# Project-MONAI/GenerativeModels

Hardware: NVIDIA H100
Metric: ddim50_voxels_per_s (higher is better)
Workload: dtype fp16

## Files before the change

generativemodels_b200/csrc/flash_attn.cu:

```cuda
#include "common.cuh"
#include "wgmma.cuh"
#include <cuda.h>
#include <cudaTypedefs.h>
#include <mutex>
#include <string.h>

namespace b200 {

struct FlashDev {
  alignas(64) CUtensorMap tmQ;
  alignas(64) CUtensorMap tmK;
  alignas(64) CUtensorMap tmVt;
  int B, T, S, heads, dh, d_chunks;
  int q_tiles, q_tiles_grid, n_items, n_kv;
  float scale_log2;
  h16* out;
  long long out_bstride, out_pitch;
  const h16* res;
  long long res_bstride, res_pitch;
};

namespace fa {

static constexpr int kThreads = 128;
static constexpr int kBM = 64, kBKV = 64;
static constexpr int kChunkBytes = 64 * 64 * 2;

__device__ __forceinline__ float ex2_approx(float x) {
  float y;
  asm("ex2.approx.ftz.f32 %0, %1;" : "=f"(y) : "f"(x));
  return y;
}
__device__ __forceinline__ uint32_t pack_h2(float lo, float hi) {
  h162 v = f2h2(lo, hi);
  return *reinterpret_cast<uint32_t*>(&v);
}

template <int DCH>
__global__ void __launch_bounds__(kThreads, 1) flash_attn_kernel(const __grid_constant__ FlashDev p) {
  constexpr int DV = 64 * DCH;
  extern __shared__ uint8_t smem_raw[];
  const uint32_t q_base = (smem_u32(smem_raw) + 1023u) & ~1023u;
  const uint32_t k_base = q_base + DCH * kChunkBytes;
  const uint32_t v_base = k_base + DCH * kChunkBytes;
  const uint32_t bar = v_base + DV * kBKV * 2;
  const uint32_t q_bar = bar, k_bar = bar + 8, v_bar = bar + 16;

  const int tid = threadIdx.x;
  const int warp = tid >> 5, lane = tid & 31;
  int x = blockIdx.x;
  const int qt = x % p.q_tiles; x /= p.q_tiles;
  const int h = x % p.heads;
  const int b = x / p.heads;
  const int q0 = qt * kBM;
  const int qc = h * p.dh;
  const int vc = qc;

  if (tid == 0) {
    mbar_init(q_bar, 1);
    mbar_init(k_bar, 1);
    mbar_init(v_bar, 1);
    asm volatile("fence.mbarrier_init.release.cluster;" ::: "memory");
    asm volatile("fence.proxy.async.shared::cta;" ::: "memory");
  }
  __syncthreads();
  if (tid == 0) {
    mbar_arrive_expect_tx(q_bar, DCH * kChunkBytes);
    for (int c = 0; c < DCH; ++c) tma_load_3d(&p.tmQ, q_bar, q_base + c * kChunkBytes, qc + 64 * c, q0, b);
    mbar_arrive_expect_tx(k_bar, DCH * kChunkBytes);
    for (int c = 0; c < DCH; ++c) tma_load_3d(&p.tmK, k_bar, k_base + c * kChunkBytes, qc + 64 * c, 0, b);
    mbar_arrive_expect_tx(v_bar, DV * kBKV * 2);
    tma_load_3d(&p.tmVt, v_bar, v_base, 0, vc, b);
  }

  float o[DV / 2];
#pragma unroll
  for (int i = 0; i < DV / 2; ++i) o[i] = 0.f;
  float m0 = -INFINITY, m1 = -INFINITY, l0 = 0.f, l1 = 0.f;
  const float sc = p.scale_log2;
  mbar_wait(q_bar, 0);

  for (int j = 0; j < p.n_kv; ++j) {
    const uint32_t ph = j & 1;
    float s[32];
    mbar_wait(k_bar, ph);
    wgmma_fence();
#pragma unroll
    for (int c = 0; c < DCH; ++c) {
      const uint64_t qd = wgmma_desc(q_base + c * kChunkBytes), kd = wgmma_desc(k_base + c * kChunkBytes);
#pragma unroll
      for (int kk = 0; kk < 4; ++kk) wgmma_ss<64>(s, qd + 2u * kk, kd + 2u * kk, (c | kk) != 0 ? 1u : 0u);
    }
    wgmma_commit();
    wgmma_wait<0>();
    wgmma_touch<32>(s);
    __syncthreads();
    if (tid == 0 && j + 1 < p.n_kv) {
      mbar_arrive_expect_tx(k_bar, DCH * kChunkBytes);
      for (int c = 0; c < DCH; ++c) tma_load_3d(&p.tmK, k_bar, k_base + c * kChunkBytes, qc + 64 * c, (j + 1) * kBKV, b);
    }

    const int key0 = j * kBKV + 2 * (lane & 3);
    float mx0 = -INFINITY, mx1 = -INFINITY;
#pragma unroll
    for (int n = 0; n < 8; ++n) {
#pragma unroll
      for (int e = 0; e < 2; ++e) {
        const bool ok = key0 + 8 * n + e < p.S;
        s[4 * n + e] = ok ? s[4 * n + e] * sc : -INFINITY;
        s[4 * n + 2 + e] = ok ? s[4 * n + 2 + e] * sc : -INFINITY;
        mx0 = fmaxf(mx0, s[4 * n + e]);
        mx1 = fmaxf(mx1, s[4 * n + 2 + e]);
      }
    }
    mx0 = fmaxf(mx0, __shfl_xor_sync(0xffffffffu, mx0, 1));
    mx0 = fmaxf(mx0, __shfl_xor_sync(0xffffffffu, mx0, 2));
    mx1 = fmaxf(mx1, __shfl_xor_sync(0xffffffffu, mx1, 1));
    mx1 = fmaxf(mx1, __shfl_xor_sync(0xffffffffu, mx1, 2));
    const float nm0 = fmaxf(m0, mx0), nm1 = fmaxf(m1, mx1);
    const float u0 = nm0 == -INFINITY ? 0.f : nm0, u1 = nm1 == -INFINITY ? 0.f : nm1;
    const float a0 = ex2_approx(m0 - u0), a1 = ex2_approx(m1 - u1);
    m0 = nm0;
    m1 = nm1;
    uint32_t pa[16];
    float ps0 = 0.f, ps1 = 0.f;
#pragma unroll
    for (int n = 0; n < 8; ++n) {
      const float p00 = ex2_approx(s[4 * n] - u0), p01 = ex2_approx(s[4 * n + 1] - u0);
      const float p10 = ex2_approx(s[4 * n + 2] - u1), p11 = ex2_approx(s[4 * n + 3] - u1);
      ps0 += p00 + p01;
      ps1 += p10 + p11;
      pa[4 * (n >> 1) + 2 * (n & 1)] = pack_h2(p00, p01);
      pa[4 * (n >> 1) + 2 * (n & 1) + 1] = pack_h2(p10, p11);
    }
    l0 = l0 * a0 + ps0;
    l1 = l1 * a1 + ps1;
#pragma unroll
    for (int n = 0; n < DV / 8; ++n) {
      o[4 * n] *= a0; o[4 * n + 1] *= a0;
      o[4 * n + 2] *= a1; o[4 * n + 3] *= a1;
    }

    mbar_wait(v_bar, ph);
    wgmma_fence();
    const uint64_t vd = wgmma_desc(v_base);
#pragma unroll
    for (int kk = 0; kk < 4; ++kk) wgmma_rs<DV>(o, pa + 4 * kk, vd + 2u * kk, 1u);
    wgmma_commit();
    wgmma_wait<0>();
    wgmma_touch<DV / 2>(o);
    __syncthreads();
    if (tid == 0 && j + 1 < p.n_kv) {
      mbar_arrive_expect_tx(v_bar, DV * kBKV * 2);
      tma_load_3d(&p.tmVt, v_bar, v_base, (j + 1) * kBKV, vc, b);
    }
  }

  l0 += __shfl_xor_sync(0xffffffffu, l0, 1);
  l0 += __shfl_xor_sync(0xffffffffu, l0, 2);
  l1 += __shfl_xor_sync(0xffffffffu, l1, 1);
  l1 += __shfl_xor_sync(0xffffffffu, l1, 2);
  const float inv0 = 1.f / l0, inv1 = 1.f / l1;
  const int r0 = 16 * warp + (lane >> 2);
#pragma unroll
  for (int half = 0; half < 2; ++half) {
    const int t = q0 + r0 + 8 * half;
    if (t >= p.T) continue;
    const float inv = half ? inv1 : inv0;
    h16* orow = p.out + (long long)b * p.out_bstride + (long long)t * p.out_pitch + vc;
    const h16* rrow = p.res ? p.res + (long long)b * p.res_bstride + (long long)t * p.res_pitch + vc : nullptr;
#pragma unroll
    for (int n = 0; n < DV / 8; ++n) {
      const int col = 8 * n + 2 * (lane & 3);
      float v0 = o[4 * n + 2 * half] * inv, v1 = o[4 * n + 2 * half + 1] * inv;
      if (rrow) {
        const float2 r = h22f2(*reinterpret_cast<const h162*>(rrow + col));
        v0 += r.x;
        v1 += r.y;
      }
      *reinterpret_cast<h162*>(orow + col) = f2h2(v0, v1);
    }
  }
}

template <int DCH>
constexpr int smem_bytes() { return 1024 + 2 * DCH * kChunkBytes + DCH * 64 * kBKV * 2 + 64; }

namespace d512 {
static constexpr int kThreads = 384;
static constexpr int kCluster = 2;
static constexpr int kBlockKeys = 128;
static constexpr int kRing = 16;
static constexpr int kChunksPerBlock = 32;
static constexpr int kOffRing = 8 * kChunkBytes;
static constexpr int kOffP = kOffRing + kRing * kChunkBytes;
static constexpr int kOffX = kOffP + 2 * kChunkBytes;
static constexpr int kOffBar = kOffX + 4 * 64 * 4;
static constexpr int kSmem = 1024 + kOffBar + (1 + 2 * kRing) * 8;
static constexpr int kProducerRegs = 40, kConsumerRegs = 232;
static_assert(kProducerRegs * 128 + kConsumerRegs * 256 <= 65536, "register budget of one CTA per SM");
}

__global__ void __launch_bounds__(d512::kThreads, 1) flash_attn_d512_kernel(const __grid_constant__ FlashDev p) {
  using namespace d512;
  extern __shared__ uint8_t smem_raw[];
  uint8_t* sm = smem_raw + ((1024u - (smem_u32(smem_raw) & 1023u)) & 1023u);
  const uint32_t base = smem_u32(sm);
  const uint32_t q_base = base, ring = base + kOffRing, p_base = base + kOffP;
  float* xmax = reinterpret_cast<float*>(sm + kOffX);
  float* xsum = xmax + 2 * 64;
  const uint32_t q_bar = base + kOffBar;
  const uint32_t full0 = q_bar + 8, empty0 = full0 + 8 * kRing;

  const int tid = threadIdx.x;
  const int wg = __shfl_sync(0xffffffffu, tid >> 7, 0);
  const uint32_t rank = cluster_ctarank();
  int x = blockIdx.x;
  const int qt = x % p.q_tiles_grid; x /= p.q_tiles_grid;
  const int h = x % p.heads;
  const int b = x / p.heads;
  const bool rows_valid = qt < p.q_tiles;
  const int q0 = (rows_valid ? qt : p.q_tiles - 1) * kBM;
  const int qc = h * 512;

  if (tid == 0) {
    mbar_init(q_bar, 1);
    for (int s = 0; s < kRing; ++s) {
      mbar_init(full0 + 8 * s, 1);
      mbar_init(empty0 + 8 * s, 4 * kCluster);
    }
    asm volatile("fence.mbarrier_init.release.cluster;" ::: "memory");
  }
  cluster_sync();

  if (wg == 0) {
    setmaxnreg_dec<kProducerRegs>();
    if (tid == 0) {
      mbar_arrive_expect_tx(q_bar, 8 * kChunkBytes);
      for (int c = 0; c < 8; ++c) tma_load_3d(&p.tmQ, q_bar, q_base + c * kChunkBytes, qc + 64 * c, q0, b);
      for (int j = 0; j < p.n_kv; ++j) {
        for (int n = 0; n < kChunksPerBlock; ++n) {
          const int slot = n % kRing;
          mbar_wait(empty0 + 8 * slot, ((n / kRing) & 1) ^ 1);
          mbar_arrive_expect_tx(full0 + 8 * slot, kChunkBytes);
          if ((n & 1) != (int)rank) continue;
          const uint32_t dst = ring + slot * kChunkBytes, fb = full0 + 8 * slot;
          if (n < 16) {
            const int d = (n & 3) | ((n >> 3) << 2);
            tma_load_3d_multicast(&p.tmK, fb, dst, qc + 64 * d, j * kBlockKeys + 64 * ((n >> 2) & 1), b, 0x3);
          } else {
            const int g = (n - 16) >> 2;
            tma_load_3d_multicast(&p.tmVt, fb, dst, j * kBlockKeys + 64 * (g >> 1), qc + 256 * (g & 1) + 64 * (n & 3), b,
                                  0x3);
          }
        }
      }
    }
  } else {
    setmaxnreg_inc<kConsumerRegs>();
    const int c = wg - 1;
    const int t = tid & 127, warp = t >> 5, lane = tid & 31, q4 = lane & 3;
    const int r0 = 16 * warp + (lane >> 2);
    const int sw = r0 & 7;
    uint32_t* pmine = reinterpret_cast<uint32_t*>(sm + kOffP + c * kChunkBytes);
    const uint64_t pd_partner = wgmma_desc(p_base + (1 - c) * kChunkBytes);
    auto release = [&](int slot) {
      if (lane == 0) {
        mbar_arrive_cluster(empty0 + 8 * slot, 0);
        mbar_arrive_cluster(empty0 + 8 * slot, 1);
      }
    };

    float o[128];
#pragma unroll
    for (int i = 0; i < 128; ++i) o[i] = 0.f;
    float m0 = -INFINITY, m1 = -INFINITY, l0 = 0.f, l1 = 0.f;
    const float sc = p.scale_log2;
    mbar_wait(q_bar, 0);

    for (int j = 0; j < p.n_kv; ++j) {
      float s[32];
      auto k_slot = [c](int d) { return (d & 3) | (c << 2) | ((d >> 2) << 3); };
#pragma unroll
      for (int d = 0; d < 8; ++d) {
        const int slot = k_slot(d);
        mbar_wait(full0 + 8 * slot, 0);
        if (d == 0) wgmma_fence();
        const uint64_t qd = wgmma_desc(q_base + d * kChunkBytes), kd = wgmma_desc(ring + slot * kChunkBytes);
#pragma unroll
        for (int kk = 0; kk < 4; ++kk) wgmma_ss<64>(s, qd + 2u * kk, kd + 2u * kk, (d | kk) != 0 ? 1u : 0u);
        wgmma_commit();
        if (d >= 2) {
          wgmma_wait<2>();
          release(k_slot(d - 2));
        }
      }
      wgmma_wait<1>();
      release(k_slot(6));
      wgmma_wait<0>();
      release(k_slot(7));
      wgmma_touch<32>(s);

      const int key0 = j * kBlockKeys + 64 * c + 2 * q4;
      float mx0 = -INFINITY, mx1 = -INFINITY;
#pragma unroll
      for (int n = 0; n < 8; ++n) {
#pragma unroll
        for (int e = 0; e < 2; ++e) {
          const bool ok = key0 + 8 * n + e < p.S;
          s[4 * n + e] = ok ? s[4 * n + e] * sc : -INFINITY;
          s[4 * n + 2 + e] = ok ? s[4 * n + 2 + e] * sc : -INFINITY;
          mx0 = fmaxf(mx0, s[4 * n + e]);
          mx1 = fmaxf(mx1, s[4 * n + 2 + e]);
        }
      }
      mx0 = fmaxf(mx0, __shfl_xor_sync(0xffffffffu, mx0, 1));
      mx0 = fmaxf(mx0, __shfl_xor_sync(0xffffffffu, mx0, 2));
      mx1 = fmaxf(mx1, __shfl_xor_sync(0xffffffffu, mx1, 1));
      mx1 = fmaxf(mx1, __shfl_xor_sync(0xffffffffu, mx1, 2));
      if (q4 == 0) {
        xmax[64 * c + r0] = mx0;
        xmax[64 * c + r0 + 8] = mx1;
      }
      named_sync(1, 256);
      mx0 = fmaxf(mx0, xmax[64 * (1 - c) + r0]);
      mx1 = fmaxf(mx1, xmax[64 * (1 - c) + r0 + 8]);
      const float nm0 = fmaxf(m0, mx0), nm1 = fmaxf(m1, mx1);
      const float u0 = nm0 == -INFINITY ? 0.f : nm0, u1 = nm1 == -INFINITY ? 0.f : nm1;
      const float a0 = ex2_approx(m0 - u0), a1 = ex2_approx(m1 - u1);
      m0 = nm0;
      m1 = nm1;
      uint32_t pa[16];
      float ps0 = 0.f, ps1 = 0.f;
#pragma unroll
      for (int n = 0; n < 8; ++n) {
        const float p00 = ex2_approx(s[4 * n] - u0), p01 = ex2_approx(s[4 * n + 1] - u0);
        const float p10 = ex2_approx(s[4 * n + 2] - u1), p11 = ex2_approx(s[4 * n + 3] - u1);
        ps0 += p00 + p01;
        ps1 += p10 + p11;
        const uint32_t lo = pack_h2(p00, p01), hi = pack_h2(p10, p11);
        pa[4 * (n >> 1) + 2 * (n & 1)] = lo;
        pa[4 * (n >> 1) + 2 * (n & 1) + 1] = hi;
        pmine[(r0 * 128 + ((n ^ sw) << 4) + 4 * q4) >> 2] = lo;
        pmine[((r0 + 8) * 128 + ((n ^ sw) << 4) + 4 * q4) >> 2] = hi;
      }
      asm volatile("fence.proxy.async.shared::cta;" ::: "memory");
      l0 = l0 * a0 + ps0;
      l1 = l1 * a1 + ps1;
#pragma unroll
      for (int n = 0; n < 32; ++n) {
        o[4 * n] *= a0; o[4 * n + 1] *= a0;
        o[4 * n + 2] *= a1; o[4 * n + 3] *= a1;
      }
      named_sync(1, 256);

#pragma unroll
      for (int hh = 0; hh < 2; ++hh) {
        const int g = 2 * hh + c;
#pragma unroll
        for (int i = 0; i < 4; ++i) mbar_wait(full0 + 8 * (4 * g + i), 1);
        if (hh == 0) wgmma_fence();
        const uint64_t vd = wgmma_desc(ring + 4 * g * kChunkBytes);
        if (hh == c) {
#pragma unroll
          for (int kk = 0; kk < 4; ++kk) wgmma_rs<256>(o, pa + 4 * kk, vd + 2u * kk, 1u);
        } else {
#pragma unroll
          for (int kk = 0; kk < 4; ++kk) wgmma_ss<256>(o, pd_partner + 2u * kk, vd + 2u * kk, 1u);
        }
        wgmma_commit();
      }
      wgmma_wait<1>();
#pragma unroll
      for (int i = 0; i < 4; ++i) release(4 * c + i);
      wgmma_wait<0>();
      wgmma_touch<128>(o);
      wgmma_touch_u32<16>(pa);
#pragma unroll
      for (int i = 0; i < 4; ++i) release(4 * (2 + c) + i);
    }

    l0 += __shfl_xor_sync(0xffffffffu, l0, 1);
    l0 += __shfl_xor_sync(0xffffffffu, l0, 2);
    l1 += __shfl_xor_sync(0xffffffffu, l1, 1);
    l1 += __shfl_xor_sync(0xffffffffu, l1, 2);
    if (q4 == 0) {
      xsum[64 * c + r0] = l0;
      xsum[64 * c + r0 + 8] = l1;
    }
    named_sync(1, 256);
    const float inv0 = 1.f / (l0 + xsum[64 * (1 - c) + r0]), inv1 = 1.f / (l1 + xsum[64 * (1 - c) + r0 + 8]);
    const int vc = qc + 256 * c;
#pragma unroll
    for (int half = 0; half < 2; ++half) {
      const int tq = q0 + r0 + 8 * half;
      if (!rows_valid || tq >= p.T) continue;
      const float inv = half ? inv1 : inv0;
      h16* orow = p.out + (long long)b * p.out_bstride + (long long)tq * p.out_pitch + vc;
      const h16* rrow = p.res ? p.res + (long long)b * p.res_bstride + (long long)tq * p.res_pitch + vc : nullptr;
#pragma unroll
      for (int n = 0; n < 32; ++n) {
        const int col = 8 * n + 2 * q4;
        float v0 = o[4 * n + 2 * half] * inv, v1 = o[4 * n + 2 * half + 1] * inv;
        if (rrow) {
          const float2 r = h22f2(*reinterpret_cast<const h162*>(rrow + col));
          v0 += r.x;
          v1 += r.y;
        }
        *reinterpret_cast<h162*>(orow + col) = f2h2(v0, v1);
      }
    }
  }
  cluster_sync();
}

static PFN_cuTensorMapEncodeTiled g_encode = nullptr;
static std::once_flag g_once;
static void load_encode() {
  void* fn = nullptr;
  cudaDriverEntryPointQueryResult qres;
  if (cudaGetDriverEntryPoint("cuTensorMapEncodeTiled", &fn, cudaEnableDefault, &qres) == cudaSuccess &&
      qres == cudaDriverEntryPointSuccess)
    g_encode = reinterpret_cast<PFN_cuTensorMapEncodeTiled>(fn);
}

static int encode3(CUtensorMap* tm, const void* ptr, cuuint64_t d0, cuuint64_t d1, cuuint64_t d2, cuuint64_t s1_bytes,
                   cuuint64_t s2_bytes, cuuint32_t b0, cuuint32_t b1, const char* what) {
  cuuint64_t dims[3] = {d0, d1, d2};
  cuuint64_t strides[2] = {s1_bytes, s2_bytes};
  cuuint32_t box[3] = {b0, b1, 1};
  cuuint32_t estr[3] = {1, 1, 1};
  CUresult r = g_encode(tm, B200_H16_TMAP, 3, const_cast<void*>(ptr), dims, strides, box, estr,
                        CU_TENSOR_MAP_INTERLEAVE_NONE, CU_TENSOR_MAP_SWIZZLE_128B, CU_TENSOR_MAP_L2_PROMOTION_L2_256B,
                        CU_TENSOR_MAP_FLOAT_OOB_FILL_NONE);
  if (r != CUDA_SUCCESS) {
    set_error("attention_flash: cuTensorMapEncodeTiled(%s) failed with %d", what, (int)r);
    return B200_ECUDA;
  }
  return B200_OK;
}

template <int DCH>
static int launch(const FlashDev& d, cudaStream_t stream) {
  constexpr int smem = smem_bytes<DCH>();
  static_assert(smem <= 227 * 1024, "attention_flash: shared memory over the 227 KB a block may use");
  static std::once_flag attr_once;
  static cudaError_t attr_rc = cudaSuccess;
  std::call_once(attr_once, [] {
    attr_rc = cudaFuncSetAttribute(flash_attn_kernel<DCH>, cudaFuncAttributeMaxDynamicSharedMemorySize, smem);
  });
  B200_CUDA(attr_rc);
  B200_CUDA(b200::launch_kernel(flash_attn_kernel<DCH>, d.n_items, kThreads, smem, stream, d));
  B200_LAUNCH_CHECK("flash_attn_kernel");
  return B200_OK;
}

static int launch_d512(const FlashDev& d, cudaStream_t stream) {
  static_assert(d512::kSmem <= 227 * 1024, "attention_flash: shared memory over the 227 KB a block may use");
  static std::once_flag attr_once;
  static cudaError_t attr_rc = cudaSuccess;
  std::call_once(attr_once, [] {
    attr_rc = cudaFuncSetAttribute(flash_attn_d512_kernel, cudaFuncAttributeMaxDynamicSharedMemorySize, d512::kSmem);
  });
  B200_CUDA(attr_rc);
  B200_CUDA(b200::launch_kernel<d512::kCluster>(flash_attn_d512_kernel, d.n_items, d512::kThreads, d512::kSmem, stream, d));
  B200_LAUNCH_CHECK("flash_attn_d512_kernel");
  return B200_OK;
}

}
}

using namespace b200;

extern "C" int64_t b200_attention_flash_workspace_bytes(const b200_flash_params* a) {
  (void)a;
  return 0;
}

extern "C" int b200_attention_flash(const b200_flash_params* a, void* stream_v) {
  cudaStream_t stream = static_cast<cudaStream_t>(stream_v);
  B200_CHECK_ARG(a && a->q && a->k && a->vt && a->out, "attention_flash: null pointer");
  B200_CHECK_ARG(a->B >= 1 && a->T >= 1 && a->S >= 1 && a->heads >= 1, "attention_flash: bad extents");
  B200_CHECK_ARG(a->dh == 64 || a->dh == 128 || a->dh == 256 || a->dh == 512,
                 "attention_flash: head_dim %d not in {64,128,256,512}", a->dh);
  B200_CHECK_ARG(a->q_pitch % 8 == 0 && a->k_pitch % 8 == 0 && a->vt_pitch % 8 == 0 && a->out_pitch % 8 == 0,
                 "attention_flash: pitches must be multiples of 8 elements");
  B200_CHECK_ARG(((uintptr_t)a->q & 15) == 0 && ((uintptr_t)a->k & 15) == 0 && ((uintptr_t)a->vt & 15) == 0 &&
                 ((uintptr_t)a->out & 15) == 0 && ((uintptr_t)a->res & 15) == 0, "attention_flash: 16-byte alignment");
  B200_CHECK_ARG(!a->res || a->res_pitch % 8 == 0, "attention_flash: residual pitch must be a multiple of 8");
  std::call_once(fa::g_once, fa::load_encode);
  if (!fa::g_encode) { set_error("attention_flash: cuTensorMapEncodeTiled unavailable"); return B200_ECUDA; }

  FlashDev d;
  memset(&d, 0, sizeof(d));
  const int C = a->heads * a->dh;
  const bool d512 = a->dh == 512;
  d.B = a->B; d.T = a->T; d.S = a->S; d.heads = a->heads; d.dh = a->dh;
  d.d_chunks = a->dh / 64;
  d.q_tiles = (a->T + fa::kBM - 1) / fa::kBM;
  d.q_tiles_grid = d512 ? (d.q_tiles + fa::d512::kCluster - 1) / fa::d512::kCluster * fa::d512::kCluster : d.q_tiles;
  const int bkv = d512 ? fa::d512::kBlockKeys : fa::kBKV;
  d.n_kv = (a->S + bkv - 1) / bkv;
  const long long items = (long long)a->B * a->heads * d.q_tiles_grid;
  B200_CHECK_ARG(items < (1ll << 31), "attention_flash: too many work items");
  d.n_items = (int)items;
  d.scale_log2 = a->scale * 1.4426950408889634f;
  d.out = reinterpret_cast<h16*>(a->out);
  d.out_pitch = a->out_pitch; d.out_bstride = (long long)a->T * a->out_pitch;
  d.res = reinterpret_cast<const h16*>(a->res);
  d.res_pitch = a->res_pitch; d.res_bstride = (long long)a->T * a->res_pitch;
  int rc;
  if ((rc = fa::encode3(&d.tmQ, a->q, C, a->T, a->B, (cuuint64_t)a->q_pitch * 2, (cuuint64_t)a->T * a->q_pitch * 2, 64,
                        fa::kBM, "Q"))) return rc;
  if ((rc = fa::encode3(&d.tmK, a->k, C, a->S, a->B, (cuuint64_t)a->k_pitch * 2, (cuuint64_t)a->S * a->k_pitch * 2, 64,
                        fa::kBKV, "K"))) return rc;
  if ((rc = fa::encode3(&d.tmVt, a->vt, a->S, C, a->B, (cuuint64_t)a->vt_pitch * 2, (cuuint64_t)C * a->vt_pitch * 2,
                        fa::kBKV, d512 ? 64 : a->dh, "V^T"))) return rc;
  switch (d.d_chunks) {
    case 1: return fa::launch<1>(d, stream);
    case 2: return fa::launch<2>(d, stream);
    case 4: return fa::launch<4>(d, stream);
    default: return fa::launch_d512(d, stream);
  }
}
```

generativemodels_b200/csrc/wgmma.cuh:

```cuda
#pragma once
#include "common.cuh"
#include <cuda.h>

#ifdef B200_H16_IS_BF16
#define B200_WGMMA_AB "bf16"
#else
#define B200_WGMMA_AB "f16"
#endif

namespace b200 {

__device__ __forceinline__ uint64_t wgmma_desc(uint32_t smem_addr) {
  uint64_t d = 0;
  d |= static_cast<uint64_t>((smem_addr & 0x3FFFFu) >> 4);
  d |= static_cast<uint64_t>(1) << 16;
  d |= static_cast<uint64_t>(1024 >> 4) << 32;
  d |= static_cast<uint64_t>(1) << 62;
  return d;
}
__device__ __forceinline__ void wgmma_fence() { asm volatile("wgmma.fence.sync.aligned;" ::: "memory"); }
__device__ __forceinline__ void wgmma_commit() { asm volatile("wgmma.commit_group.sync.aligned;" ::: "memory"); }
template <int N>
__device__ __forceinline__ void wgmma_wait() { asm volatile("wgmma.wait_group.sync.aligned %0;" ::"n"(N) : "memory"); }
template <int R>
__device__ __forceinline__ void wgmma_touch(float* d) {
#pragma unroll
  for (int i = 0; i < R; ++i) asm volatile("" : "+f"(d[i])::"memory");
}

__device__ __forceinline__ void wgmma_ss_n16(float* d, uint64_t adesc, uint64_t bdesc, uint32_t accumulate) {
  asm volatile(
      "{\n\t.reg .pred p;\n\t"
      "setp.ne.b32 p, %10, 0;\n\t"
      "wgmma.mma_async.sync.aligned.m64n16k16.f32." B200_WGMMA_AB "." B200_WGMMA_AB " "
      "{%0, %1, %2, %3, %4, %5, %6, %7}, %8, %9, p, 1, 1, 0, 0;\n\t}"
      : "+f"(d[0]), "+f"(d[1]), "+f"(d[2]), "+f"(d[3]), "+f"(d[4]), "+f"(d[5]), "+f"(d[6]), "+f"(d[7])
      : "l"(adesc), "l"(bdesc), "r"(accumulate));
}

__device__ __forceinline__ void wgmma_ss_n32(float* d, uint64_t adesc, uint64_t bdesc, uint32_t accumulate) {
  asm volatile(
      "{\n\t.reg .pred p;\n\t"
      "setp.ne.b32 p, %18, 0;\n\t"
      "wgmma.mma_async.sync.aligned.m64n32k16.f32." B200_WGMMA_AB "." B200_WGMMA_AB " "
      "{%0, %1, %2, %3, %4, %5, %6, %7, %8, %9, %10, %11, %12, %13, %14, %15}, %16, %17, p, 1, 1, 0, 0;\n\t}"
      : "+f"(d[0]), "+f"(d[1]), "+f"(d[2]), "+f"(d[3]), "+f"(d[4]), "+f"(d[5]), "+f"(d[6]), "+f"(d[7]), "+f"(d[8]), "+f"(d[9]), "+f"(d[10]), "+f"(d[11]), "+f"(d[12]), "+f"(d[13]), "+f"(d[14]), "+f"(d[15])
      : "l"(adesc), "l"(bdesc), "r"(accumulate));
}

__device__ __forceinline__ void wgmma_ss_n64(float* d, uint64_t adesc, uint64_t bdesc, uint32_t accumulate) {
  asm volatile(
      "{\n\t.reg .pred p;\n\t"
      "setp.ne.b32 p, %34, 0;\n\t"
      "wgmma.mma_async.sync.aligned.m64n64k16.f32." B200_WGMMA_AB "." B200_WGMMA_AB " "
      "{%0, %1, %2, %3, %4, %5, %6, %7, %8, %9, %10, %11, %12, %13, %14, %15, %16, %17, %18, %19, %20, %21, %22, %23, %24, %25, %26, %27, %28, %29, %30, %31}, %32, %33, p, 1, 1, 0, 0;\n\t}"
      : "+f"(d[0]), "+f"(d[1]), "+f"(d[2]), "+f"(d[3]), "+f"(d[4]), "+f"(d[5]), "+f"(d[6]), "+f"(d[7]), "+f"(d[8]), "+f"(d[9]), "+f"(d[10]), "+f"(d[11]), "+f"(d[12]), "+f"(d[13]), "+f"(d[14]), "+f"(d[15]), "+f"(d[16]), "+f"(d[17]), "+f"(d[18]), "+f"(d[19]), "+f"(d[20]), "+f"(d[21]), "+f"(d[22]), "+f"(d[23]), "+f"(d[24]), "+f"(d[25]), "+f"(d[26]), "+f"(d[27]), "+f"(d[28]), "+f"(d[29]), "+f"(d[30]), "+f"(d[31])
      : "l"(adesc), "l"(bdesc), "r"(accumulate));
}

__device__ __forceinline__ void wgmma_ss_n128(float* d, uint64_t adesc, uint64_t bdesc, uint32_t accumulate) {
  asm volatile(
      "{\n\t.reg .pred p;\n\t"
      "setp.ne.b32 p, %66, 0;\n\t"
      "wgmma.mma_async.sync.aligned.m64n128k16.f32." B200_WGMMA_AB "." B200_WGMMA_AB " "
      "{%0, %1, %2, %3, %4, %5, %6, %7, %8, %9, %10, %11, %12, %13, %14, %15, %16, %17, %18, %19, %20, %21, %22, %23, %24, %25, %26, %27, %28, %29, %30, %31, %32, %33, %34, %35, %36, %37, %38, %39, %40, %41, %42, %43, %44, %45, %46, %47, %48, %49, %50, %51, %52, %53, %54, %55, %56, %57, %58, %59, %60, %61, %62, %63}, %64, %65, p, 1, 1, 0, 0;\n\t}"
      : "+f"(d[0]), "+f"(d[1]), "+f"(d[2]), "+f"(d[3]), "+f"(d[4]), "+f"(d[5]), "+f"(d[6]), "+f"(d[7]), "+f"(d[8]), "+f"(d[9]), "+f"(d[10]), "+f"(d[11]), "+f"(d[12]), "+f"(d[13]), "+f"(d[14]), "+f"(d[15]), "+f"(d[16]), "+f"(d[17]), "+f"(d[18]), "+f"(d[19]), "+f"(d[20]), "+f"(d[21]), "+f"(d[22]), "+f"(d[23]), "+f"(d[24]), "+f"(d[25]), "+f"(d[26]), "+f"(d[27]), "+f"(d[28]), "+f"(d[29]), "+f"(d[30]), "+f"(d[31]), "+f"(d[32]), "+f"(d[33]), "+f"(d[34]), "+f"(d[35]), "+f"(d[36]), "+f"(d[37]), "+f"(d[38]), "+f"(d[39]), "+f"(d[40]), "+f"(d[41]), "+f"(d[42]), "+f"(d[43]), "+f"(d[44]), "+f"(d[45]), "+f"(d[46]), "+f"(d[47]), "+f"(d[48]), "+f"(d[49]), "+f"(d[50]), "+f"(d[51]), "+f"(d[52]), "+f"(d[53]), "+f"(d[54]), "+f"(d[55]), "+f"(d[56]), "+f"(d[57]), "+f"(d[58]), "+f"(d[59]), "+f"(d[60]), "+f"(d[61]), "+f"(d[62]), "+f"(d[63])
      : "l"(adesc), "l"(bdesc), "r"(accumulate));
}

__device__ __forceinline__ void wgmma_ss_n256(float* d, uint64_t adesc, uint64_t bdesc, uint32_t accumulate) {
  asm volatile(
      "{\n\t.reg .pred p;\n\t"
      "setp.ne.b32 p, %130, 0;\n\t"
      "wgmma.mma_async.sync.aligned.m64n256k16.f32." B200_WGMMA_AB "." B200_WGMMA_AB " "
      "{%0, %1, %2, %3, %4, %5, %6, %7, %8, %9, %10, %11, %12, %13, %14, %15, %16, %17, %18, %19, %20, %21, %22, %23, %24, %25, %26, %27, %28, %29, %30, %31, %32, %33, %34, %35, %36, %37, %38, %39, %40, %41, %42, %43, %44, %45, %46, %47, %48, %49, %50, %51, %52, %53, %54, %55, %56, %57, %58, %59, %60, %61, %62, %63, %64, %65, %66, %67, %68, %69, %70, %71, %72, %73, %74, %75, %76, %77, %78, %79, %80, %81, %82, %83, %84, %85, %86, %87, %88, %89, %90, %91, %92, %93, %94, %95, %96, %97, %98, %99, %100, %101, %102, %103, %104, %105, %106, %107, %108, %109, %110, %111, %112, %113, %114, %115, %116, %117, %118, %119, %120, %121, %122, %123, %124, %125, %126, %127}, %128, %129, p, 1, 1, 0, 0;\n\t}"
      : "+f"(d[0]), "+f"(d[1]), "+f"(d[2]), "+f"(d[3]), "+f"(d[4]), "+f"(d[5]), "+f"(d[6]), "+f"(d[7]), "+f"(d[8]), "+f"(d[9]), "+f"(d[10]), "+f"(d[11]), "+f"(d[12]), "+f"(d[13]), "+f"(d[14]), "+f"(d[15]), "+f"(d[16]), "+f"(d[17]), "+f"(d[18]), "+f"(d[19]), "+f"(d[20]), "+f"(d[21]), "+f"(d[22]), "+f"(d[23]), "+f"(d[24]), "+f"(d[25]), "+f"(d[26]), "+f"(d[27]), "+f"(d[28]), "+f"(d[29]), "+f"(d[30]), "+f"(d[31]), "+f"(d[32]), "+f"(d[33]), "+f"(d[34]), "+f"(d[35]), "+f"(d[36]), "+f"(d[37]), "+f"(d[38]), "+f"(d[39]), "+f"(d[40]), "+f"(d[41]), "+f"(d[42]), "+f"(d[43]), "+f"(d[44]), "+f"(d[45]), "+f"(d[46]), "+f"(d[47]), "+f"(d[48]), "+f"(d[49]), "+f"(d[50]), "+f"(d[51]), "+f"(d[52]), "+f"(d[53]), "+f"(d[54]), "+f"(d[55]), "+f"(d[56]), "+f"(d[57]), "+f"(d[58]), "+f"(d[59]), "+f"(d[60]), "+f"(d[61]), "+f"(d[62]), "+f"(d[63]), "+f"(d[64]), "+f"(d[65]), "+f"(d[66]), "+f"(d[67]), "+f"(d[68]), "+f"(d[69]), "+f"(d[70]), "+f"(d[71]), "+f"(d[72]), "+f"(d[73]), "+f"(d[74]), "+f"(d[75]), "+f"(d[76]), "+f"(d[77]), "+f"(d[78]), "+f"(d[79]), "+f"(d[80]), "+f"(d[81]), "+f"(d[82]), "+f"(d[83]), "+f"(d[84]), "+f"(d[85]), "+f"(d[86]), "+f"(d[87]), "+f"(d[88]), "+f"(d[89]), "+f"(d[90]), "+f"(d[91]), "+f"(d[92]), "+f"(d[93]), "+f"(d[94]), "+f"(d[95]), "+f"(d[96]), "+f"(d[97]), "+f"(d[98]), "+f"(d[99]), "+f"(d[100]), "+f"(d[101]), "+f"(d[102]), "+f"(d[103]), "+f"(d[104]), "+f"(d[105]), "+f"(d[106]), "+f"(d[107]), "+f"(d[108]), "+f"(d[109]), "+f"(d[110]), "+f"(d[111]), "+f"(d[112]), "+f"(d[113]), "+f"(d[114]), "+f"(d[115]), "+f"(d[116]), "+f"(d[117]), "+f"(d[118]), "+f"(d[119]), "+f"(d[120]), "+f"(d[121]), "+f"(d[122]), "+f"(d[123]), "+f"(d[124]), "+f"(d[125]), "+f"(d[126]), "+f"(d[127])
      : "l"(adesc), "l"(bdesc), "r"(accumulate));
}

template <int N>
__device__ __forceinline__ void wgmma_ss(float* d, uint64_t adesc, uint64_t bdesc, uint32_t accumulate) {
  if constexpr (N == 16) wgmma_ss_n16(d, adesc, bdesc, accumulate);
  else if constexpr (N == 32) wgmma_ss_n32(d, adesc, bdesc, accumulate);
  else if constexpr (N == 64) wgmma_ss_n64(d, adesc, bdesc, accumulate);
  else if constexpr (N == 128) wgmma_ss_n128(d, adesc, bdesc, accumulate);
  else wgmma_ss_n256(d, adesc, bdesc, accumulate);
}

template <int R>
__device__ __forceinline__ void wgmma_touch_u32(uint32_t* a) {
#pragma unroll
  for (int i = 0; i < R; ++i) asm volatile("" : "+r"(a[i])::"memory");
}

template <int N>
__device__ __forceinline__ void setmaxnreg_dec() { asm volatile("setmaxnreg.dec.sync.aligned.u32 %0;" ::"n"(N)); }
template <int N>
__device__ __forceinline__ void setmaxnreg_inc() { asm volatile("setmaxnreg.inc.sync.aligned.u32 %0;" ::"n"(N)); }

__device__ __forceinline__ void wgmma_rs_n64(float* d, const uint32_t* a, uint64_t bdesc, uint32_t accumulate) {
  asm volatile(
      "{\n\t.reg .pred p;\n\t"
      "setp.ne.b32 p, %37, 0;\n\t"
      "wgmma.mma_async.sync.aligned.m64n64k16.f32." B200_WGMMA_AB "." B200_WGMMA_AB " "
      "{%0, %1, %2, %3, %4, %5, %6, %7, %8, %9, %10, %11, %12, %13, %14, %15, %16, %17, %18, %19, %20, %21, %22, %23, %24, %25, %26, %27, %28, %29, %30, %31}, {%32, %33, %34, %35}, %36, p, 1, 1, 0;\n\t}"
      : "+f"(d[0]), "+f"(d[1]), "+f"(d[2]), "+f"(d[3]), "+f"(d[4]), "+f"(d[5]), "+f"(d[6]), "+f"(d[7]), "+f"(d[8]), "+f"(d[9]), "+f"(d[10]), "+f"(d[11]), "+f"(d[12]), "+f"(d[13]), "+f"(d[14]), "+f"(d[15]), "+f"(d[16]), "+f"(d[17]), "+f"(d[18]), "+f"(d[19]), "+f"(d[20]), "+f"(d[21]), "+f"(d[22]), "+f"(d[23]), "+f"(d[24]), "+f"(d[25]), "+f"(d[26]), "+f"(d[27]), "+f"(d[28]), "+f"(d[29]), "+f"(d[30]), "+f"(d[31])
      : "r"(a[0]), "r"(a[1]), "r"(a[2]), "r"(a[3]), "l"(bdesc), "r"(accumulate));
}

__device__ __forceinline__ void wgmma_rs_n128(float* d, const uint32_t* a, uint64_t bdesc, uint32_t accumulate) {
  asm volatile(
      "{\n\t.reg .pred p;\n\t"
      "setp.ne.b32 p, %69, 0;\n\t"
      "wgmma.mma_async.sync.aligned.m64n128k16.f32." B200_WGMMA_AB "." B200_WGMMA_AB " "
      "{%0, %1, %2, %3, %4, %5, %6, %7, %8, %9, %10, %11, %12, %13, %14, %15, %16, %17, %18, %19, %20, %21, %22, %23, %24, %25, %26, %27, %28, %29, %30, %31, %32, %33, %34, %35, %36, %37, %38, %39, %40, %41, %42, %43, %44, %45, %46, %47, %48, %49, %50, %51, %52, %53, %54, %55, %56, %57, %58, %59, %60, %61, %62, %63}, {%64, %65, %66, %67}, %68, p, 1, 1, 0;\n\t}"
      : "+f"(d[0]), "+f"(d[1]), "+f"(d[2]), "+f"(d[3]), "+f"(d[4]), "+f"(d[5]), "+f"(d[6]), "+f"(d[7]), "+f"(d[8]), "+f"(d[9]), "+f"(d[10]), "+f"(d[11]), "+f"(d[12]), "+f"(d[13]), "+f"(d[14]), "+f"(d[15]), "+f"(d[16]), "+f"(d[17]), "+f"(d[18]), "+f"(d[19]), "+f"(d[20]), "+f"(d[21]), "+f"(d[22]), "+f"(d[23]), "+f"(d[24]), "+f"(d[25]), "+f"(d[26]), "+f"(d[27]), "+f"(d[28]), "+f"(d[29]), "+f"(d[30]), "+f"(d[31]), "+f"(d[32]), "+f"(d[33]), "+f"(d[34]), "+f"(d[35]), "+f"(d[36]), "+f"(d[37]), "+f"(d[38]), "+f"(d[39]), "+f"(d[40]), "+f"(d[41]), "+f"(d[42]), "+f"(d[43]), "+f"(d[44]), "+f"(d[45]), "+f"(d[46]), "+f"(d[47]), "+f"(d[48]), "+f"(d[49]), "+f"(d[50]), "+f"(d[51]), "+f"(d[52]), "+f"(d[53]), "+f"(d[54]), "+f"(d[55]), "+f"(d[56]), "+f"(d[57]), "+f"(d[58]), "+f"(d[59]), "+f"(d[60]), "+f"(d[61]), "+f"(d[62]), "+f"(d[63])
      : "r"(a[0]), "r"(a[1]), "r"(a[2]), "r"(a[3]), "l"(bdesc), "r"(accumulate));
}

__device__ __forceinline__ void wgmma_rs_n256(float* d, const uint32_t* a, uint64_t bdesc, uint32_t accumulate) {
  asm volatile(
      "{\n\t.reg .pred p;\n\t"
      "setp.ne.b32 p, %133, 0;\n\t"
      "wgmma.mma_async.sync.aligned.m64n256k16.f32." B200_WGMMA_AB "." B200_WGMMA_AB " "
      "{%0, %1, %2, %3, %4, %5, %6, %7, %8, %9, %10, %11, %12, %13, %14, %15, %16, %17, %18, %19, %20, %21, %22, %23, %24, %25, %26, %27, %28, %29, %30, %31, %32, %33, %34, %35, %36, %37, %38, %39, %40, %41, %42, %43, %44, %45, %46, %47, %48, %49, %50, %51, %52, %53, %54, %55, %56, %57, %58, %59, %60, %61, %62, %63, %64, %65, %66, %67, %68, %69, %70, %71, %72, %73, %74, %75, %76, %77, %78, %79, %80, %81, %82, %83, %84, %85, %86, %87, %88, %89, %90, %91, %92, %93, %94, %95, %96, %97, %98, %99, %100, %101, %102, %103, %104, %105, %106, %107, %108, %109, %110, %111, %112, %113, %114, %115, %116, %117, %118, %119, %120, %121, %122, %123, %124, %125, %126, %127}, {%128, %129, %130, %131}, %132, p, 1, 1, 0;\n\t}"
      : "+f"(d[0]), "+f"(d[1]), "+f"(d[2]), "+f"(d[3]), "+f"(d[4]), "+f"(d[5]), "+f"(d[6]), "+f"(d[7]), "+f"(d[8]), "+f"(d[9]), "+f"(d[10]), "+f"(d[11]), "+f"(d[12]), "+f"(d[13]), "+f"(d[14]), "+f"(d[15]), "+f"(d[16]), "+f"(d[17]), "+f"(d[18]), "+f"(d[19]), "+f"(d[20]), "+f"(d[21]), "+f"(d[22]), "+f"(d[23]), "+f"(d[24]), "+f"(d[25]), "+f"(d[26]), "+f"(d[27]), "+f"(d[28]), "+f"(d[29]), "+f"(d[30]), "+f"(d[31]), "+f"(d[32]), "+f"(d[33]), "+f"(d[34]), "+f"(d[35]), "+f"(d[36]), "+f"(d[37]), "+f"(d[38]), "+f"(d[39]), "+f"(d[40]), "+f"(d[41]), "+f"(d[42]), "+f"(d[43]), "+f"(d[44]), "+f"(d[45]), "+f"(d[46]), "+f"(d[47]), "+f"(d[48]), "+f"(d[49]), "+f"(d[50]), "+f"(d[51]), "+f"(d[52]), "+f"(d[53]), "+f"(d[54]), "+f"(d[55]), "+f"(d[56]), "+f"(d[57]), "+f"(d[58]), "+f"(d[59]), "+f"(d[60]), "+f"(d[61]), "+f"(d[62]), "+f"(d[63]), "+f"(d[64]), "+f"(d[65]), "+f"(d[66]), "+f"(d[67]), "+f"(d[68]), "+f"(d[69]), "+f"(d[70]), "+f"(d[71]), "+f"(d[72]), "+f"(d[73]), "+f"(d[74]), "+f"(d[75]), "+f"(d[76]), "+f"(d[77]), "+f"(d[78]), "+f"(d[79]), "+f"(d[80]), "+f"(d[81]), "+f"(d[82]), "+f"(d[83]), "+f"(d[84]), "+f"(d[85]), "+f"(d[86]), "+f"(d[87]), "+f"(d[88]), "+f"(d[89]), "+f"(d[90]), "+f"(d[91]), "+f"(d[92]), "+f"(d[93]), "+f"(d[94]), "+f"(d[95]), "+f"(d[96]), "+f"(d[97]), "+f"(d[98]), "+f"(d[99]), "+f"(d[100]), "+f"(d[101]), "+f"(d[102]), "+f"(d[103]), "+f"(d[104]), "+f"(d[105]), "+f"(d[106]), "+f"(d[107]), "+f"(d[108]), "+f"(d[109]), "+f"(d[110]), "+f"(d[111]), "+f"(d[112]), "+f"(d[113]), "+f"(d[114]), "+f"(d[115]), "+f"(d[116]), "+f"(d[117]), "+f"(d[118]), "+f"(d[119]), "+f"(d[120]), "+f"(d[121]), "+f"(d[122]), "+f"(d[123]), "+f"(d[124]), "+f"(d[125]), "+f"(d[126]), "+f"(d[127])
      : "r"(a[0]), "r"(a[1]), "r"(a[2]), "r"(a[3]), "l"(bdesc), "r"(accumulate));
}

template <int N>
__device__ __forceinline__ void wgmma_rs(float* d, const uint32_t* a, uint64_t bdesc, uint32_t accumulate) {
  if constexpr (N == 64) wgmma_rs_n64(d, a, bdesc, accumulate);
  else if constexpr (N == 128) wgmma_rs_n128(d, a, bdesc, accumulate);
  else wgmma_rs_n256(d, a, bdesc, accumulate);
}

__device__ __forceinline__ uint32_t smem_u32(const void* p) {
  return static_cast<uint32_t>(__cvta_generic_to_shared(p));
}
__device__ __forceinline__ void mbar_init(uint32_t bar, uint32_t count) {
  asm volatile("mbarrier.init.shared::cta.b64 [%0], %1;" ::"r"(bar), "r"(count));
}
__device__ __forceinline__ void mbar_arrive_expect_tx(uint32_t bar, uint32_t bytes) {
  asm volatile("mbarrier.arrive.expect_tx.shared::cta.b64 _, [%0], %1;" ::"r"(bar), "r"(bytes) : "memory");
}
__device__ __forceinline__ void mbar_arrive(uint32_t bar) {
  asm volatile("mbarrier.arrive.shared::cta.b64 _, [%0];" ::"r"(bar) : "memory");
}
__device__ __forceinline__ void mbar_wait(uint32_t bar, uint32_t parity) {
  uint32_t done;
  do {
    asm volatile(
        "{\n\t.reg .pred p;\n\t"
        "mbarrier.try_wait.parity.shared::cta.b64 p, [%1], %2;\n\t"
        "selp.u32 %0, 1, 0, p;\n\t}"
        : "=r"(done)
        : "r"(bar), "r"(parity)
        : "memory");
  } while (!done);
}
__device__ __forceinline__ void mbar_arrive_cluster(uint32_t bar, uint32_t cta) {
  uint32_t remote;
  asm volatile("mapa.shared::cluster.u32 %0, %1, %2;" : "=r"(remote) : "r"(bar), "r"(cta));
  asm volatile("mbarrier.arrive.shared::cluster.b64 _, [%0];" ::"r"(remote) : "memory");
}
__device__ __forceinline__ void tma_load_3d(const CUtensorMap* tm, uint32_t bar, uint32_t dst, int c0, int c1, int c2) {
  asm volatile(
      "cp.async.bulk.tensor.3d.shared::cluster.global.mbarrier::complete_tx::bytes"
      " [%0], [%1, {%3, %4, %5}], [%2];" ::"r"(dst),
      "l"(reinterpret_cast<uint64_t>(tm)), "r"(bar), "r"(c0), "r"(c1), "r"(c2)
      : "memory");
}
__device__ __forceinline__ void tma_load_3d_multicast(const CUtensorMap* tm, uint32_t bar, uint32_t dst, int c0, int c1,
                                                      int c2, uint16_t cta_mask) {
  asm volatile(
      "cp.async.bulk.tensor.3d.shared::cluster.global.mbarrier::complete_tx::bytes.multicast::cluster"
      " [%0], [%1, {%3, %4, %5}], [%2], %6;" ::"r"(dst),
      "l"(reinterpret_cast<uint64_t>(tm)), "r"(bar), "r"(c0), "r"(c1), "r"(c2), "h"(cta_mask)
      : "memory");
}
__device__ __forceinline__ uint32_t cluster_ctarank() {
  uint32_t r;
  asm volatile("mov.u32 %0, %%cluster_ctarank;" : "=r"(r));
  return r;
}
__device__ __forceinline__ void cluster_sync() {
  asm volatile("barrier.cluster.arrive.release.aligned;\n\tbarrier.cluster.wait.acquire.aligned;" ::: "memory");
}
__device__ __forceinline__ void named_sync(uint32_t id, uint32_t threads) {
  asm volatile("bar.sync %0, %1;" ::"r"(id), "r"(threads) : "memory");
}

}
```

Before: 146,300.

## Alternate full-block QK^T between consumer warpgroups to overlap softmax with PV

Before, both consumer warpgroups each computed half of every 128-key S block and exchanged row maxima through shared memory every iteration. Now each warpgroup owns alternating KV blocks, computing the full 64x128 S tile and its softmax. It writes P and the new max/partial sums to shared memory for the partner, which only rescales and runs PV. The producer now issues K loads two blocks ahead with per-consumer full barriers, so one group's QK^T and softmax can overlap the other's PV. This adds named-barrier handoffs and a larger S register array (64 floats) at the 232-register budget, which risks spills or stalls.

```diff
diff --git a/generativemodels_b200/csrc/flash_attn.cu b/generativemodels_b200/csrc/flash_attn.cu
--- a/generativemodels_b200/csrc/flash_attn.cu
+++ b/generativemodels_b200/csrc/flash_attn.cu
@@ -191,14 +191,14 @@
 static constexpr int kCluster = 2;
 static constexpr int kBlockKeys = 128;
 static constexpr int kRing = 16;
-static constexpr int kChunksPerBlock = 32;
 static constexpr int kOffRing = 8 * kChunkBytes;
 static constexpr int kOffP = kOffRing + kRing * kChunkBytes;
 static constexpr int kOffX = kOffP + 2 * kChunkBytes;
-static constexpr int kOffBar = kOffX + 4 * 64 * 4;
-static constexpr int kSmem = 1024 + kOffBar + (1 + 2 * kRing) * 8;
+static constexpr int kOffBar = kOffX + 2048;
+static constexpr int kSmem = 1024 + kOffBar + (1 + 3 * kRing) * 8;
 static constexpr int kProducerRegs = 40, kConsumerRegs = 232;
 static_assert(kProducerRegs * 128 + kConsumerRegs * 256 <= 65536, "register budget of one CTA per SM");
+static constexpr uint32_t kBarReady = 1, kBarFree = 3, kBarTile = 5, kBarSums = 7;
 }
 
 __global__ void __launch_bounds__(d512::kThreads, 1) flash_attn_d512_kernel(const __grid_constant__ FlashDev p) {
@@ -208,27 +208,29 @@
   const uint32_t base = smem_u32(sm);
   const uint32_t q_base = base, ring = base + kOffRing, p_base = base + kOffP;
   float* xmax = reinterpret_cast<float*>(sm + kOffX);
-  float* xsum = xmax + 2 * 64;
+  float* xps = xmax + 64;
+  float* xsum = xps + 2 * 128;
   const uint32_t q_bar = base + kOffBar;
-  const uint32_t full0 = q_bar + 8, empty0 = full0 + 8 * kRing;
+  const uint32_t full0 = q_bar + 8, empty0 = full0 + 2 * 8 * kRing;
 
   const int tid = threadIdx.x;
   const int wg = __shfl_sync(0xffffffffu, tid >> 7, 0);
-  const uint32_t rank = cluster_ctarank();
-  int x = blockIdx.x;
-  const int qt = x % p.q_tiles_grid; x /= p.q_tiles_grid;
-  const int h = x % p.heads;
-  const int b = x / p.heads;
-  const bool rows_valid = qt < p.q_tiles;
-  const int q0 = (rows_valid ? qt : p.q_tiles - 1) * kBM;
-  const int qc = h * 512;
+  const int n_kv = p.n_kv;
+  struct Item { int qt, b, q0, qc; };
+  auto item = [&]() {
+    Item it;
+    int x = blockIdx.x;
+    it.qt = x % p.q_tiles_grid; x /= p.q_tiles_grid;
+    it.qc = (x % p.heads) * 512;
+    it.b = x / p.heads;
+    it.q0 = (it.qt < p.q_tiles ? it.qt : p.q_tiles - 1) * kBM;
+    return it;
+  };
 
   if (tid == 0) {
     mbar_init(q_bar, 1);
-    for (int s = 0; s < kRing; ++s) {
-      mbar_init(full0 + 8 * s, 1);
-      mbar_init(empty0 + 8 * s, 4 * kCluster);
-    }
+    for (int s = 0; s < 2 * kRing; ++s) mbar_init(full0 + 8 * s, 1);
+    for (int s = 0; s < kRing; ++s) mbar_init(empty0 + 8 * s, 4 * kCluster);
     asm volatile("fence.mbarrier_init.release.cluster;" ::: "memory");
   }
   cluster_sync();
@@ -236,24 +238,32 @@
   if (wg == 0) {
     setmaxnreg_dec<kProducerRegs>();
     if (tid == 0) {
+      const uint32_t rank = cluster_ctarank();
+      const Item it = item();
+      const int b = it.b, qc = it.qc;
       mbar_arrive_expect_tx(q_bar, 8 * kChunkBytes);
-      for (int c = 0; c < 8; ++c) tma_load_3d(&p.tmQ, q_bar, q_base + c * kChunkBytes, qc + 64 * c, q0, b);
-      for (int j = 0; j < p.n_kv; ++j) {
-        for (int n = 0; n < kChunksPerBlock; ++n) {
-          const int slot = n % kRing;
-          mbar_wait(empty0 + 8 * slot, ((n / kRing) & 1) ^ 1);
-          mbar_arrive_expect_tx(full0 + 8 * slot, kChunkBytes);
-          if ((n & 1) != (int)rank) continue;
-          const uint32_t dst = ring + slot * kChunkBytes, fb = full0 + 8 * slot;
-          if (n < 16) {
-            const int d = (n & 3) | ((n >> 3) << 2);
-            tma_load_3d_multicast(&p.tmK, fb, dst, qc + 64 * d, j * kBlockKeys + 64 * ((n >> 2) & 1), b, 0x3);
-          } else {
-            const int g = (n - 16) >> 2;
-            tma_load_3d_multicast(&p.tmVt, fb, dst, j * kBlockKeys + 64 * (g >> 1), qc + 256 * (g & 1) + 64 * (n & 3), b,
-                                  0x3);
-          }
+      for (int c = 0; c < 8; ++c) tma_load_3d(&p.tmQ, q_bar, q_base + c * kChunkBytes, qc + 64 * c, it.q0, b);
+      uint32_t unit = 0;
+      auto emit = [&](int j, bool vt) {
+        for (int i = 0; i < kRing; ++i) {
+          mbar_wait(empty0 + 8 * i, (unit & 1) ^ 1);
+          const int reader = vt ? (i >> 2) & 1 : j & 1;
+          const uint32_t fb = full0 + 8 * (kRing * reader + i), dst = ring + i * kChunkBytes;
+          mbar_arrive_expect_tx(fb, kChunkBytes);
+          if ((i & 1) != (int)rank) continue;
+          if (vt)
+            tma_load_3d_multicast(&p.tmVt, fb, dst, j * kBlockKeys + 64 * (i >> 3), qc + 256 * ((i >> 2) & 1) + 64 * (i & 3),
+                                  b, 0x3);
+          else
+            tma_load_3d_multicast(&p.tmK, fb, dst, qc + 64 * (i >> 1), j * kBlockKeys + 64 * (i & 1), b, 0x3);
         }
+        ++unit;
+      };
+      emit(0, false);
+      if (n_kv > 1) emit(1, false);
+      for (int j = 0; j < n_kv; ++j) {
+        emit(j, true);
+        if (j + 2 < n_kv) emit(j + 2, false);
       }
     }
   } else {
@@ -262,49 +272,85 @@
     const int t = tid & 127, warp = t >> 5, lane = tid & 31, q4 = lane & 3;
     const int r0 = 16 * warp + (lane >> 2);
     const int sw = r0 & 7;
-    uint32_t* pmine = reinterpret_cast<uint32_t*>(sm + kOffP + c * kChunkBytes);
-    const uint64_t pd_partner = wgmma_desc(p_base + (1 - c) * kChunkBytes);
+    uint32_t* ptile = reinterpret_cast<uint32_t*>(sm + kOffP);
+    const uint32_t fullc = full0 + 8 * kRing * c;
+    uint32_t fph = 0;
+    auto wait_full = [&](int slot) {
+      mbar_wait(fullc + 8 * slot, (fph >> slot) & 1);
+      fph ^= 1u << slot;
+    };
     auto release = [&](int slot) {
       if (lane == 0) {
         mbar_arrive_cluster(empty0 + 8 * slot, 0);
         mbar_arrive_cluster(empty0 + 8 * slot, 1);
       }
     };
+    auto release_group = [&](int g) {
+#pragma unroll
+      for (int i = 0; i < 4; ++i) release(4 * g + i);
+    };
 
     float o[128];
 #pragma unroll
     for (int i = 0; i < 128; ++i) o[i] = 0.f;
+    float s[64];
     float m0 = -INFINITY, m1 = -INFINITY, l0 = 0.f, l1 = 0.f;
     const float sc = p.scale_log2;
-    mbar_wait(q_bar, 0);
-
-    for (int j = 0; j < p.n_kv; ++j) {
-      float s[32];
-      auto k_slot = [c](int d) { return (d & 3) | (c << 2) | ((d >> 2) << 3); };
+
+    auto issue_s = [&]() {
 #pragma unroll
       for (int d = 0; d < 8; ++d) {
-        const int slot = k_slot(d);
-        mbar_wait(full0 + 8 * slot, 0);
+        wait_full(2 * d);
+        wait_full(2 * d + 1);
         if (d == 0) wgmma_fence();
-        const uint64_t qd = wgmma_desc(q_base + d * kChunkBytes), kd = wgmma_desc(ring + slot * kChunkBytes);
-#pragma unroll
-        for (int kk = 0; kk < 4; ++kk) wgmma_ss<64>(s, qd + 2u * kk, kd + 2u * kk, (d | kk) != 0 ? 1u : 0u);
+        const uint64_t qd = wgmma_desc(q_base + d * kChunkBytes), kd = wgmma_desc(ring + 2 * d * kChunkBytes);
+#pragma unroll
+        for (int kk = 0; kk < 4; ++kk) wgmma_ss<128>(s, qd + 2u * kk, kd + 2u * kk, (d | kk) != 0 ? 1u : 0u);
         wgmma_commit();
         if (d >= 2) {
           wgmma_wait<2>();
-          release(k_slot(d - 2));
+          release(2 * d - 4);
+          release(2 * d - 3);
         }
       }
       wgmma_wait<1>();
-      release(k_slot(6));
+      release(12);
+      release(13);
       wgmma_wait<0>();
-      release(k_slot(7));
-      wgmma_touch<32>(s);
-
-      const int key0 = j * kBlockKeys + 64 * c + 2 * q4;
+      release(14);
+      release(15);
+      wgmma_touch<64>(s);
+    };
+    auto issue_pv = [&]() {
+#pragma unroll
+      for (int hh = 0; hh < 2; ++hh) {
+        const int g = 2 * hh + c;
+#pragma unroll
+        for (int i = 0; i < 4; ++i) wait_full(4 * g + i);
+        if (hh == 0) wgmma_fence();
+        const uint64_t vd = wgmma_desc(ring + 4 * g * kChunkBytes), pd = wgmma_desc(p_base + hh * kChunkBytes);
+#pragma unroll
+        for (int kk = 0; kk < 4; ++kk) wgmma_ss<256>(o, pd + 2u * kk, vd + 2u * kk, 1u);
+        wgmma_commit();
+      }
+    };
+
+    mbar_wait(q_bar, 0);
+    if (c < n_kv) issue_s();
+
+    auto owner = [&](int j) {
+      wgmma_wait<1>();
+      if (j > 0) release_group(c);
+      wgmma_wait<0>();
+      wgmma_touch<128>(o);
+      if (j > 0) {
+        release_group(2 + c);
+        named_sync(kBarFree + (c ^ 1), 256);
+      }
+      const int key0 = j * kBlockKeys + 2 * q4;
       float mx0 = -INFINITY, mx1 = -INFINITY;
 #pragma unroll
-      for (int n = 0; n < 8; ++n) {
+      for (int n = 0; n < 16; ++n) {
 #pragma unroll
         for (int e = 0; e < 2; ++e) {
           const bool ok = key0 + 8 * n + e < p.S;
@@ -318,67 +364,79 @@
       mx0 = fmaxf(mx0, __shfl_xor_sync(0xffffffffu, mx0, 2));
       mx1 = fmaxf(mx1, __shfl_xor_sync(0xffffffffu, mx1, 1));
       mx1 = fmaxf(mx1, __shfl_xor_sync(0xffffffffu, mx1, 2));
-      if (q4 == 0) {
-        xmax[64 * c + r0] = mx0;
-        xmax[64 * c + r0 + 8] = mx1;
-      }
-      named_sync(1, 256);
-      mx0 = fmaxf(mx0, xmax[64 * (1 - c) + r0]);
-      mx1 = fmaxf(mx1, xmax[64 * (1 - c) + r0 + 8]);
       const float nm0 = fmaxf(m0, mx0), nm1 = fmaxf(m1, mx1);
       const float u0 = nm0 == -INFINITY ? 0.f : nm0, u1 = nm1 == -INFINITY ? 0.f : nm1;
       const float a0 = ex2_approx(m0 - u0), a1 = ex2_approx(m1 - u1);
       m0 = nm0;
       m1 = nm1;
-      uint32_t pa[16];
-      float ps0 = 0.f, ps1 = 0.f;
-#pragma unroll
-      for (int n = 0; n < 8; ++n) {
+      float ps00 = 0.f, ps01 = 0.f, ps10 = 0.f, ps11 = 0.f;
+#pragma unroll
+      for (int n = 0; n < 16; ++n) {
         const float p00 = ex2_approx(s[4 * n] - u0), p01 = ex2_approx(s[4 * n + 1] - u0);
         const float p10 = ex2_approx(s[4 * n + 2] - u1), p11 = ex2_approx(s[4 * n + 3] - u1);
-        ps0 += p00 + p01;
-        ps1 += p10 + p11;
-        const uint32_t lo = pack_h2(p00, p01), hi = pack_h2(p10, p11);
-        pa[4 * (n >> 1) + 2 * (n & 1)] = lo;
-        pa[4 * (n >> 1) + 2 * (n & 1) + 1] = hi;
-        pmine[(r0 * 128 + ((n ^ sw) << 4) + 4 * q4) >> 2] = lo;
-        pmine[((r0 + 8) * 128 + ((n ^ sw) << 4) + 4 * q4) >> 2] = hi;
-      }
+        if (n < 8) {
+          ps00 += p00 + p01;
+          ps01 += p10 + p11;
+        } else {
+          ps10 += p00 + p01;
+          ps11 += p10 + p11;
+        }
+        const int nn = n & 7, tile = (n >> 3) * (kChunkBytes / 4);
+        ptile[tile + ((r0 * 128 + ((nn ^ sw) << 4) + 4 * q4) >> 2)] = pack_h2(p00, p01);
+        ptile[tile + (((r0 + 8) * 128 + ((nn ^ sw) << 4) + 4 * q4) >> 2)] = pack_h2(p10, p11);
+      }
+      if (q4 == 0) {
+        xmax[r0] = nm0;
+        xmax[r0 + 8] = nm1;
+      }
+      xps[2 * t] = c ? ps00 : ps10;
+      xps[2 * t + 1] = c ? ps01 : ps11;
       asm volatile("fence.proxy.async.shared::cta;" ::: "memory");
-      l0 = l0 * a0 + ps0;
-      l1 = l1 * a1 + ps1;
+      named_arrive(kBarReady + c, 256);
+      named_sync(kBarTile + c, 128);
+      l0 = l0 * a0 + (c ? ps10 : ps00);
+      l1 = l1 * a1 + (c ? ps11 : ps01);
 #pragma unroll
       for (int n = 0; n < 32; ++n) {
         o[4 * n] *= a0; o[4 * n + 1] *= a0;
         o[4 * n + 2] *= a1; o[4 * n + 3] *= a1;
       }
-      named_sync(1, 256);
-
-#pragma unroll
-      for (int hh = 0; hh < 2; ++hh) {
-        const int g = 2 * hh + c;
-#pragma unroll
-        for (int i = 0; i < 4; ++i) mbar_wait(full0 + 8 * (4 * g + i), 1);
-        if (hh == 0) wgmma_fence();
-        const uint64_t vd = wgmma_desc(ring + 4 * g * kChunkBytes);
-        if (hh == c) {
-#pragma unroll
-          for (int kk = 0; kk < 4; ++kk) wgmma_rs<256>(o, pa + 4 * kk, vd + 2u * kk, 1u);
-        } else {
-#pragma unroll
-          for (int kk = 0; kk < 4; ++kk) wgmma_ss<256>(o, pd_partner + 2u * kk, vd + 2u * kk, 1u);
-        }
-        wgmma_commit();
-      }
+      issue_pv();
       wgmma_wait<1>();
-#pragma unroll
-      for (int i = 0; i < 4; ++i) release(4 * c + i);
+      release_group(c);
       wgmma_wait<0>();
       wgmma_touch<128>(o);
-      wgmma_touch_u32<16>(pa);
-#pragma unroll
-      for (int i = 0; i < 4; ++i) release(4 * (2 + c) + i);
-    }
+      release_group(2 + c);
+      if (j + 1 < n_kv) named_arrive(kBarFree + c, 256);
+      if (j + 2 < n_kv) issue_s();
+    };
+    auto partner = [&](int j) {
+      named_sync(kBarReady + (c ^ 1), 256);
+      const float nm0 = xmax[r0], nm1 = xmax[r0 + 8];
+      const float u0 = nm0 == -INFINITY ? 0.f : nm0, u1 = nm1 == -INFINITY ? 0.f : nm1;
+      const float a0 = ex2_approx(m0 - u0), a1 = ex2_approx(m1 - u1);
+      m0 = nm0;
+      m1 = nm1;
+      l0 = l0 * a0 + xps[2 * t];
+      l1 = l1 * a1 + xps[2 * t + 1];
+#pragma unroll
+      for (int n = 0; n < 32; ++n) {
+        o[4 * n] *= a0; o[4 * n + 1] *= a0;
+        o[4 * n + 2] *= a1; o[4 * n + 3] *= a1;
+      }
+      issue_pv();
+    };
+
+    if (c == 1) partner(0);
+    for (int j = c; j < n_kv; j += 2) {
+      owner(j);
+      if (j + 1 < n_kv) partner(j + 1);
+    }
+    wgmma_wait<1>();
+    if (((n_kv - 1) & 1) != c) release_group(c);
+    wgmma_wait<0>();
+    if (((n_kv - 1) & 1) != c) release_group(2 + c);
+    wgmma_touch<128>(o);
 
     l0 += __shfl_xor_sync(0xffffffffu, l0, 1);
     l0 += __shfl_xor_sync(0xffffffffu, l0, 2);
@@ -388,13 +446,14 @@
       xsum[64 * c + r0] = l0;
       xsum[64 * c + r0 + 8] = l1;
     }
-    named_sync(1, 256);
+    named_sync(kBarSums, 256);
     const float inv0 = 1.f / (l0 + xsum[64 * (1 - c) + r0]), inv1 = 1.f / (l1 + xsum[64 * (1 - c) + r0 + 8]);
-    const int vc = qc + 256 * c;
+    const Item it = item();
+    const int b = it.b, vc = it.qc + 256 * c;
 #pragma unroll
     for (int half = 0; half < 2; ++half) {
-      const int tq = q0 + r0 + 8 * half;
-      if (!rows_valid || tq >= p.T) continue;
+      const int tq = it.q0 + r0 + 8 * half;
+      if (it.qt >= p.q_tiles || tq >= p.T) continue;
       const float inv = half ? inv1 : inv0;
       h16* orow = p.out + (long long)b * p.out_bstride + (long long)tq * p.out_pitch + vc;
       const h16* rrow = p.res ? p.res + (long long)b * p.res_bstride + (long long)tq * p.res_pitch + vc : nullptr;
diff --git a/generativemodels_b200/csrc/wgmma.cuh b/generativemodels_b200/csrc/wgmma.cuh
--- a/generativemodels_b200/csrc/wgmma.cuh
+++ b/generativemodels_b200/csrc/wgmma.cuh
@@ -190,5 +190,8 @@
 __device__ __forceinline__ void named_sync(uint32_t id, uint32_t threads) {
   asm volatile("bar.sync %0, %1;" ::"r"(id), "r"(threads) : "memory");
 }
+__device__ __forceinline__ void named_arrive(uint32_t id, uint32_t threads) {
+  asm volatile("bar.arrive %0, %1;" ::"r"(id), "r"(threads) : "memory");
+}
 
 }
```

Result: faster. 148,800 (median of 6 runs) (+1.7%).
